# jrl-umi3218/jrl-walkgen

Hardware: AMD Instinct MI355X
Metric: QP-MPC ticks/sec (batch=4096, N=16) (higher is better)
Workload: dtype f64

## Files before the change

### include/wg_mpc.h

```cpp
#ifndef WG_MPC_H
#define WG_MPC_H

#include <stddef.h>

#ifdef __cplusplus
extern "C" {
#endif

#define WG_OK 0
#define WG_ERR_NO_DEVICE (-1)
#define WG_ERR_BAD_ARG (-2)
#define WG_ERR_HIP (-3)
#define WG_ERR_TOO_LARGE (-4)
#define WG_ERR_BUSY (-5)


int wg_init(int device_ordinal);
void wg_shutdown(void);
const char *wg_last_error(void);
int wg_abi_version(void);
size_t wg_qp_lds_bytes(int n, int m);

int wg_shard_range(long long total, int rank, int world, long long *lo, long long *hi);

// ... 88 lines not shown
  wg_foot_sample_t lf[WG_SAMPLES_PER_TICK], rf[WG_SAMPLES_PER_TICK];
  wg_foot_sample_t lf_back, rf_back;
  double pad_[15];
} wg_tick_out_t;

void wg_model_defaults(wg_model_t *model);

void wg_gait_init(const wg_model_t *model, wg_gait_state_t *state,
                  const double com0[3] , const double left_xyt[3],
                  const double right_xyt[3] );


int wg_mpc_configure(const wg_model_t *model);
int wg_mpc_reserve(int max_gaits);

int wg_mpc_tick_batch(int B, wg_gait_state_t *states, wg_tick_out_t *outs, int *diag, int advance_calls,
                      int *hist, int hist_cap, int *hist_len);
int wg_mpc_tick_batch_dev(int B, wg_gait_state_t *states, wg_tick_out_t *outs, int *diag, int advance_calls,
                          int *hist, int hist_cap, int *hist_len, void *hip_stream);
int wg_mpc_run_batch_dev(int B, wg_gait_state_t *states, int n_ticks, int advance_calls, wg_tick_out_t *outs, int *diag,
                         void *hip_stream);
int wg_mpc_run_sched_dev(int B, wg_gait_state_t *states, int n_ticks, int advance_calls, const double *vref_sched,
                         int period, wg_tick_out_t *outs, int *diag, void *hip_stream);
int wg_mpc_set_velref_dev(int B, wg_gait_state_t *states, const double *vref, void *hip_stream);
int wg_host_alloc(void **out, size_t bytes);
void wg_host_free(void *p);
int wg_mpc_tick_pinned(wg_gait_state_t *state, wg_tick_out_t *out, int *diag, int advance_calls);
int wg_mpc_assemble_batch(int B, const wg_gait_state_t *states, int advance_calls, int nmax, int mmax, double *C, double *d,
                          double *A, double *b, double *xl, double *xu, int *n, int *m);
int wg_mpc_assemble_batch_dev(int B, const wg_gait_state_t *states, int advance_calls, int nmax, int mmax, double *C, double *d,
                              double *A, double *b, double *xl, double *xu, int *n, int *m, void *hip_stream);
size_t wg_mpc_tick_lds_bytes(void);
size_t wg_mpc_tick_lds_bytes_for(const wg_model_t *model);

#define WG_RICCATI_WITH_INITIALPOS 0
#define WG_RICCATI_WITHOUT_INITIALPOS 1
int wg_riccati_solve(int n, const double *A, const double *b, const double *c, double Q, double R, int Nl, int mode,
                     double *K, double *F);
int wg_riccati_gains(double T, double zc, double Q, double R, int Nl, int mode, double *K, double *F);

#define WG_PLDP_N 16
#define WG_PLDP_MMAX (8 * WG_PLDP_N)
#define WG_PLDP_ACTIVE_CAP 40
#define WG_PLDP_NAN (-1)
#define WG_PLDP_NEG_ALPHA (-2)
#define WG_PLDP_CAPACITY (-3)
#define WG_PLDP_BAD_INPUT (-4)
typedef struct wg_pldp_state {
  int n_prev;
  int prev_active[WG_PLDP_MMAX];
  int pad_;
  double prev_zmp[2 * WG_PLDP_N];
  double internal_time;
} wg_pldp_state_t;
int wg_pldp_configure(int N, const double *iPu, const double *Px, const double *Pu);
int wg_pldp_solve_batch(int B, int mcap, const int *m, const double *D, const double *A, const double *b,
                        const double *zmpref, const double *xkyk, const int *similar, const int *n_removed,
                        const int *starting, int max_iter, wg_pldp_state_t *states, double *X, int *ret, int *n_iter,
                        int *active, int *n_active);
int wg_pldp_solve_batch_dev(int B, int mcap, const int *m, const double *D, const double *A, const double *b,
                            const double *zmpref, const double *xkyk, const int *similar, const int *n_removed,
                            const int *starting, int max_iter, wg_pldp_state_t *states, double *X, int *ret,
                            int *n_iter, int *active, int *n_active, void *hip_stream);
size_t wg_pldp_lds_bytes(void);

#define WG_POLY_MAX_ROWS 8
// ... 250 lines not shown
```

### jrl-walkgen_amd/csrc/wg_capi.hip

```cpp
#include <hip/hip_runtime.h>

#include <climits>
#include <cmath>
#include <cstdarg>
#include <cstdio>
#include <cstdlib>
#include <cstring>
#include <limits>
#include <memory>
#include <mutex>
#include <string>
#include <type_traits>
#include <vector>

#include "../../include/wg_mpc.h"
#include "wg_ql_device.hpp"
#include "wg_tick_device.hpp"
#include "wg_tick_kernels.hpp"
#include "wg_pldp_device.hpp"
#include "wg_dimitrov_device.hpp"
#include "wg_preview_device.hpp"
#include "wg_gramian_device.hpp"
#include "wg_zmpdisc_device.hpp"
#include "wg_footcons_device.hpp"
// ... 591 lines not shown
  const size_t lds = TickPlan(*model).lds;
  if (lds > 160 * 1024) return fail(WG_ERR_TOO_LARGE, "tick needs %zu B of LDS > 160 KiB", lds);
  std::vector<double> qb;
  if (model->flags & (WG_FLAG_GRAMIAN_MFMA_F64 | WG_FLAG_GRAMIAN_MFMA_F32)) {
    qb.resize((size_t)model->N * model->N);
    const int prec = (model->flags & WG_FLAG_GRAMIAN_MFMA_F32) ? WG_GRAMIAN_F32 : WG_GRAMIAN_F64;
    if (int rc = wg_gramian_batch_ctx(ctx, 1, model->N, &model->T, &model->com_height_qp, model->alpha, model->beta, model->gamma,
                                  prec, qb.data()))
      return rc;
  }
  std::lock_guard<std::mutex> lk(ctx->mu);
  std::unique_ptr<wg::TickTables> host_tables_p(new wg::TickTables);
  wg::TickTables &host_tables = *host_tables_p;
  wg::build_tables(*model, host_tables, qb.empty() ? nullptr : qb.data());
  if (!host_tables.blocks_ok && !qb.empty())
    return fail(WG_ERR_BAD_ARG, "the matrix-core Gramian is not positive definite enough for ql0002's factorisation");
  if (!ctx->tables_dev) HIP_TRY(hipMalloc(reinterpret_cast<void **>(&ctx->tables_dev), sizeof(wg::TickTables)));
  if (!ctx->model_dev) HIP_TRY(hipMalloc(reinterpret_cast<void **>(&ctx->model_dev), sizeof(wg_model_t)));
  if (int rc = ctx_wait_own(ctx)) return rc;
  HostScope hs(ctx);
  WG_H2D(ctx->tables_dev, &host_tables, sizeof host_tables);
  WG_H2D(ctx->model_dev, model, sizeof(wg_model_t));
  WG_HOST_WAIT();
  ctx->model = *model;
  ctx->model_set = true;
  return WG_OK;
}

size_t wg_mpc_tick_lds_bytes_for(const wg_model_t *model) {
  if (!model || model->N < 2 || model->N > wg::kNMaxH || tick_max_prw_steps(*model) > wg::kSMax) return 0;
  return TickPlan(*model).lds;
}

size_t wg_mpc_tick_lds_bytes_ctx(wg_ctx_t *ctx) {
  if (!ctx || !ctx->model_set) return 0;
  return TickPlan(ctx->model).lds;
}

int wg_mpc_reserve_ctx(wg_ctx_t *ctx, int max_gaits) {
  if (int rc = use_ctx(ctx)) return rc;
  if (!ctx->model_set) return fail(WG_ERR_BAD_ARG, "wg_mpc_configure() has not been called on this context");
  if (max_gaits < 1) return fail(WG_ERR_BAD_ARG, "max_gaits = %d", max_gaits);
  const TickPlan plan(ctx->model);
  std::lock_guard<std::mutex> launch_lk(ctx->launch_mu);
  double *zs = nullptr;
  if (int rc = plan.reserve_slots(ctx, max_gaits, &zs)) return rc;
  return ctx->run_buf.reserve(run_buf_bytes(max_gaits));
}

}
namespace {
int tick_launch(wg_ctx_t *ctx, int B, wg_gait_state_t *states, wg_tick_out_t *outs, int *diag, int advance_calls, int *hist, int hist_cap, int *hist_len, void *hip_stream, wg_gait_state_t *host_states, int *host_done) {
  if (int rc = tick_check(ctx, B, states)) return rc;
  if (hist && (!hist_len || hist_cap <= 0)) return fail(WG_ERR_BAD_ARG, "hist needs hist_len and hist_cap > 0");
  if (B == 0) return WG_OK;
  const TickPlan plan(ctx->model);
  if (int rc = plan.raise_lds(WG_KERNEL_BY_VIEW(wg_mpc_tick_kernel, plan.view))) return rc;
  const int grid = B;
  hipStream_t st = reinterpret_cast<hipStream_t>(hip_stream);
  std::lock_guard<std::mutex> launch_lk(ctx->launch_mu);
  if (int rc = slot_claim(ctx, ctx->guard_order, st, "tick / run")) return rc;
  double *zs = nullptr;
  if (int rc = plan.reserve_slots(ctx, grid, &zs)) return rc;
  int *order = nullptr, *iters_out = nullptr;
  if (B > ctx->num_cu * plan.per_cu() && !host_states && env_flag("WG_TICK_LPT", true))
    if (int rc = lpt_prepare(ctx->tick_lpt, states, B, st, &order, &iters_out)) return rc;
// ... 961 lines not shown
```

### jrl-walkgen_amd/csrc/wg_dimitrov_device.hpp

```cpp
#pragma once
#include "wg_pldp_device.hpp"

namespace wg {

struct DimitrovConst {
  int N, solver;
  double T, Tctrl, h;
  double OptB[2 * WG_PLDP_N * 6], OptC[2 * WG_PLDP_N * 2 * WG_PLDP_N], iLQ[2 * WG_PLDP_N * 2 * WG_PLDP_N];
  PldpModel pldp;
  double Qq[2 * WG_PLDP_N * 2 * WG_PLDP_N], OptBq[2 * WG_PLDP_N * 6], OptCq[2 * WG_PLDP_N * 2 * WG_PLDP_N], PuTq[WG_PLDP_N * WG_PLDP_N];
};

struct DimitrovHost {
  static void matmul(const double *A, const double *B, double *C, int r, int inner, int c) {
    for (int i = 0; i < r; i++)
      for (int j = 0; j < c; j++) {
        double s = 0.0;
        for (int k = 0; k < inner; k++) s += A[i * inner + k] * B[k * c + j];
        C[i * c + j] = s;
      }
  }
  static bool build(const wg_dimitrov_model_t &m, DimitrovConst &K) {
    const unsigned N = (unsigned)m.N, n = 2 * N;
    const double T = m.T;
// ... 179 lines not shown
      const double cy0 = xk[3] + t * xk[4] + 0.5 * t * t * xk[5] + t * t * t * jy / 6.0;
      const double cy1 = xk[4] + t * xk[5] + 0.5 * t * t * jy;
      const double cy2 = xk[5] + t * jy;
      out->com_x[lane][0] = cx0; out->com_x[lane][1] = cx1; out->com_x[lane][2] = cx2;
      out->com_y[lane][0] = cy0; out->com_y[lane][1] = cy1; out->com_y[lane][2] = cy2;
      out->zmp_x[lane] = 1.0 * cx0 + 0.0 * cx1 + c02 * cx2;
      out->zmp_y[lane] = 1.0 * cy0 + 0.0 * cy1 + c02 * cy2;
    }
    if (lane < 2) {
      const double T = K.T;
      const double A01 = T, A02 = T * T / 2.0, A12 = T, B0 = T * T * T / 6.0, B1 = T * T / 2.0, B2 = T;
      const double u = lane == 0 ? jx : jy;
      const double *c = xk + 3 * lane;
      const double n0 = 0.0 + 1.0 * c[0] + A01 * c[1] + A02 * c[2];
      const double n1 = 0.0 + 0.0 * c[0] + 1.0 * c[1] + A12 * c[2];
      const double n2 = 0.0 + 0.0 * c[0] + 0.0 * c[1] + 1.0 * c[2];
      st->xk[3 * lane + 0] = n0 + u * B0; st->xk[3 * lane + 1] = n1 + u * B1; st->xk[3 * lane + 2] = n2 + u * B2;
    }
  }
  if (lane == 0) {
    st->starting = 0;
    st->n_removed = first_rows;
    if (out) { out->jerk_x = jx; out->jerk_y = jy; out->ret = rc; out->n_iter = it; out->n_active = S; out->m = m; }
  }
  WG_WSYNC();
  return it;
}

template <bool kLQ>
struct DimitrovQldProb {
  static constexpr bool kCompact = false;
  static constexpr bool kNanExact = WG_TICK_NAN_EXACT != 0;
  static constexpr bool kHasFactor = false;
  static constexpr bool kRowOps = false;
  static constexpr bool kWideN = false;
  static constexpr int kFixedLdz = 0;
  static constexpr int kNM = 2 * WG_PLDP_N;
  const wg_zmp_polytope_t *polys;
  const int *slot;
  const int *rowbase;
  const double *PuT;
  int N;
  __device__ __forceinline__ double coef(int k, int inst, int axis) const { return polys[inst].A[k - rowbase[inst]][axis]; }
  __device__ __forceinline__ double G(const QlView &q, int i, int j) const {
    if constexpr (kLQ) return i == j ? q.Gdiag[i] : 0.0;
    else {
      const double g = q.G[i + j * q.ldg], dg = q.Gdiag[i];
      return i == j ? dg : g;
    }
  }
  __device__ __forceinline__ double Gd(const QlView &q, int i) const { return q.Gdiag[i]; }
  __device__ __forceinline__ void setGd(const QlView &q, int i, double v) const { q.Gdiag[i] = v; }
  __device__ __forceinline__ double xl(const QlView &, int) const { return -1e8; }
  __device__ __forceinline__ double xu(const QlView &, int) const { return 1e8; }
  __device__ __forceinline__ double A(const QlView &, int k, int i) const {
    const bool second = i >= N;
    const int kk = second ? i - N : i;
    const int inst = slot[k];
    const double a = coef(k, inst, second ? 1 : 0);
    if constexpr (kLQ) return a * PuT[kk * N + inst];
    else {
      const double pu = PuT[kk * N + (kk <= inst ? inst : kk)];
      return kk <= inst ? a * pu : 0.0;
    }
  }
  static constexpr bool kRegRows = true;
// ... 147 lines not shown
```

### jrl-walkgen_amd/csrc/wg_ql_device.hpp

```cpp
#pragma once
#include <hip/hip_runtime.h>

#include <type_traits>

#include "wg_wave.hpp"
#include "wg_ql_view.hpp"
#include "wg_ql_phases.hpp"

namespace wg {

#define WG_BACKSUB(q, s, nact, lane)                                                                   \
  do {                                                                                                 \
    if constexpr (P::kNM > 0 && P::kNM + 12 <= 48) backsub_lds<48>(q, s, nact, lane, q.sc0);          \
    else if (P::kNM == 0 && (P::kWideN || q.n >= 48) && (nact) <= 60) backsub_lds<96>(q, s, nact, lane, q.sc0);     \
    else if (P::kNM == 0 && !P::kRowOps && q.n >= 24 && (nact) <= 36) backsub_lds<48>(q, s, nact, lane, q.sc0); \
    else backsub(q, s, nact, lane);                                                                    \
  } while (0)
#define WG_SWEEP(q, s, nu, nact, lane) \
  do { if (P::kNM > 0 || (!P::kRowOps && q.n <= 64)) sweep_flat<P::kFixedLdz>(q, s, nu, nact, lane PT_SW_ARG); else sweep<(P::kRowOps ? WG_ELEM_GRP : 8), P::kWideN>(q, s, nu, nact, lane); } while (0)

#define QL_SCAN_ACCEPT                                                                        \
  if (wak <= 0.0) continue;                                                                   \
  double sumx = -sum * wak;                                                                   \
  if (k + 1 <= me) sumx = fabs(sumx);                                                         \
// ... 16 lines not shown
  const int maxit = (m + n) * 40;
  const double onha = 1.5, xmagr = .01, diagr = 2.0;
  const int ifinc = 3, kfinc = n > 10 ? n : 10;
  int jfinc = -kfinc;
  double xmag = 0.0, vfact = 1.0, res = 0.0, ratio = 0.0, diag = 0.0;
  double wsel = 1.0;
  int knext = 0;
  const int s_tail = q.r_tail;
  double *s = q.R + s_tail;
  bool early_exit = false;
  bool cap_hit = false;
  bool x_suspect = false;
  auto x_has_non_numbers = [&]() {
    bool b = false;
    for (int i = lane; i < n; i += 64) { const bool bi = !wg_sane(q.x[i]); b = b || bi; }
    return __ballot(b) != 0ull;
  };
  PT_DECL
  if (resuming) {
    nact = rs->nact; info = rs->info; iterc = rs->iterc; itref = rs->itref; iflag = rs->iflag; jfinc = rs->jfinc; knext = rs->knext;
    out.hist_len = rs->hist_len;
    xmag = rs->xmag; vfact = rs->vfact; res = rs->res; ratio = rs->ratio; diag = rs->diag;
    if constexpr (kNan) x_suspect = x_has_non_numbers();
  }

#define LOG_EVENT(code)                                                   \
  do {                                                                    \
    if (lane == 0 && hist && out.hist_len < hist_cap) hist[out.hist_len] = (code); \
    out.hist_len++;                                                       \
  } while (0)

  if (!resuming) {
    int fatal = 0x7fffffff;
    if constexpr (P::kCompact) {
      fatal = prob.norms(q, lane);
    } else {
      for (int k = lane; k < m; k += 64) {
        double sum = 0.0;
        if constexpr (P::kRowOps) sum = prob.row_sqnorm(q, k);
        else {
          WG_UNROLL
          for (int i = 0; i < n; ++i) { double a = Am(k, i); sum += a * a; }
        }
        if (sum > 0.0) sum = 1.0 / sqrt(sum);
        else if (q.b[k] == 0.0) {}
        else if (k + 1 <= me || !(q.b[k] <= 0.0)) fatal = k + 1 < fatal ? k + 1 : fatal;
        q.wa[k] = sum;
      }
    }
    for (int k = lane; k < n; k += 64) q.wa[m + k] = 1.0;
    fatal = uni(wave_min_int(fatal));
    if (fatal != 0x7fffffff) { info = -fatal; early_exit = true; }
  }
  PT(PS_NORMS);

  if (!early_exit && !resuming) {
    for (int i = lane; i < n; i += 64) q.wd[i] = prob.Gd(q, i);
    WG_WSYNC();
    if constexpr (P::kCompact) {
      diag = prob.diag_check(q, vsmall, lane);
    } else {
      double dl = 0.0;
      for (int i = lane; i < n; i += 64) {
        double wdi = q.wd[i];
        dl = maxd(dl, vsmall - wdi);
        WG_UNROLL
        for (int j = i + 1; j < n; ++j) {
          double gjj = q.wd[j], gij = Gm(i, j);
          double ga = -mind(wdi, gjj);
          double gb = fabs(wdi - gjj) + fabs(gij);
          if (gb > 0.0) ga += gij * gij / gb;
          dl = maxd(dl, ga);
        }
      }
      diag = wave_max(dl);
    }
    diag = uni(diag);
    bool need_shift = !(diag <= 0.0);
    PT(PS_DIAGCHK);
    bool factored = false;
    if constexpr (P::kHasFactor) {
      WG_REP(8)
      if (!need_shift && prob.blocks_ok) factored = WG_UBOOL(prob.factor(q, vsmall, lane));
    }
    if constexpr (P::kNM > 0 && P::kNM <= 64 && !P::kHasFactor) {
      if (!factored && !need_shift) factored = chol_inverse_regs<P::kNM>(q, prob, vsmall, lane);
    }
    if (!factored) {
    for (;;) {
      if (need_shift) {
        diag = diagr * diag;
        for (int i = lane; i < n; i += 64) prob.setGd(q, i, diag + q.wd[i]);
        WG_WSYNC();
      }
      int jfail = -1;
      double tfail = 0.0;
      for (int i = 0; i < n; ++i) {
        for (int j = i + lane; j < n; j += 64) {
          double temp = Gm(i, j);
          WG_UNROLL
          for (int k = 0; k < i; ++k) temp -= Rf(k, j) * Rf(k, i);
          if (j == i) {
            if (temp < vsmall) { q.slot[0] = 1.0; q.slot[1] = temp; }
            else { q.slot[0] = 0.0; Rf(i, i) = sqrt(temp); }
          } else q.sc0[j] = temp;
        }
        WG_WSYNC();
        if (WG_UBOOL(q.slot[0] != 0.0)) { jfail = i; tfail = q.slot[1]; break; }
// ... 653 lines not shown
```

### jrl-walkgen_amd/csrc/wg_ql_herdt.hpp

```cpp
#pragma once
#include "wg_ql_device.hpp"

namespace wg {

constexpr int kSMaxQ = 4;
constexpr int kGvLd = 4;
constexpr int kQbLd = 32;

template <int NH, int NS>
__device__ __forceinline__ bool herdt_border_rows(const QlView &q, const double *gd, const double *Gv, double vsmall, int lane) {
  constexpr int M2 = 2 * NH;
  const int i = lane;
  const bool jerk = i < NH, foot = i >= NH && i < NH + NS, row = jerk || foot;
  const int fi = i - NH;
  const int gi = jerk ? i : M2 + (foot ? fi : 0);
  double acc[NS];
#pragma unroll
  for (int f = 0; f < NS; ++f)
    acc[f] = (jerk || (foot && f >= fi)) ? ((foot && f == fi) ? gd[gi] : Gv[gi * kGvLd + f]) : 0.0;
  const double dreg = jerk ? Rf(i, i) : 1.0;
  const int colbase = jerk ? i * (i + 1) / 2 : 0;
  const int khi = jerk ? i : 0;
  double rnext = (0 < khi) ? q.Rf[colbase] : 0.0;
  for (int k = 0; k < NH; ++k) {
// ... 138 lines not shown
#pragma unroll
  for (int t = 0; t < TZ; ++t) { const int e = lane + 64 * t; zv[t] = e < NH * NH ? Z2[(e % NH) + (e / NH) * M2] : 0.0; }
#pragma unroll
  for (int t = 0; t < TR; ++t) {
    const int e = lane + 64 * t;
    if (e < NR) {
      int j = 0;
      while ((j + 1) * (j + 2) / 2 <= e) ++j;
      const int i = e - j * (j + 1) / 2;
      q.Rf[e] = rv[t];
      Rf(NH + i, NH + j) = rv[t];
    }
  }
  for (int e = lane; e < NH * NH; e += 64) { const int i = e % NH, j = NH + e / NH; Rf(i, j) = 0.0; }
#pragma unroll
  for (int t = 0; t < TZ; ++t) {
    const int e = lane + 64 * t;
    if (e < NH * NH) {
      const int i = e % NH, j = e / NH;
      Zm(i, j) = zv[t]; Zm(NH + i, NH + j) = zv[t];
      Zm(NH + i, j) = 0.0;
      Zm(i, NH + j) = ((z2sign[e >> 6] >> (e & 63)) & 1ull) ? wg_kconst(-0.0) : 0.0;
    }
  }
  for (int e = lane; e < (n - M2) * M2; e += 64) { const int i = M2 + e % (n - M2), j = e / (n - M2); Zm(i, j) = 0.0; }
}

template <int NH>
struct HerdtProb {
  static constexpr bool kCompact = true;
  static constexpr bool kNanExact = WG_TICK_NAN_EXACT != 0;
  static constexpr bool kHasFactor = true;
  static constexpr bool kRowOps = false;
  static constexpr int kNM = 2 * NH + 2 * 2;
  static constexpr int kCopRows = 4 * NH;
  static constexpr bool kWideN = false;
  static constexpr int kFixedLdz = kNM | 1;
  static_assert(4 * NH == 64, "one CoP row per lane needs 4N == 64");
  const double *Qb;
  const double *u;
  double *Gv;
  double *gd;
  const double *rowA, *rowB;
  const int *rowK, *stepidx;
  const double *V_f;
  const double *R2, *Z2;
  const unsigned long long *z2sign;
  double diag_b;
  int blocks_ok;
  int ns;
  double ax[NH], ay[NH];
  int fj;
  double ra, rb;
  double bcop;
  double ga, gb; int gk;
  __device__ __forceinline__ double fa() const { return ra + 0.0; }
  __device__ __forceinline__ double fb() const { return rb + 0.0; }
  struct FootRow { double v[4]; int c[4]; };
  __device__ __forceinline__ FootRow foot_row() const {
    const bool used = gk >= 0, pred = gk > 0;
    const int kk = used ? gk : 0;
    FootRow r;
    const int c1 = 2 * NH + kk, c3 = 2 * NH + ns + kk;
    r.c[0] = used ? (pred ? c1 - 1 : c1) : 2 * NH; r.c[1] = used ? c1 : 2 * NH;
    r.c[2] = used ? (pred ? c3 - 1 : c3) : 2 * NH; r.c[3] = used ? c3 : 2 * NH;
    r.v[0] = pred ? ga + 0.0 : 0.0; r.v[1] = used ? 0.0 - ga : 0.0;
// ... 310 lines not shown
  __device__ __forceinline__ void zt_row(const QlView &q, double *s, int rk, int lane) const {
    const int n = q.n;
    if (lane < n) {
      const int i = lane;
      const double *zc = q.Z + i * q.ldz;
      double acc = 0.0;
      if (rk >= 1 && rk <= 4 * NH) {
        constexpr int kZtChunk = 8;
        const int r = (rk - 1) >> 2;
#pragma unroll
        for (int j0 = 0; j0 < 2 * NH; j0 += kZtChunk) {
          if ((j0 < NH ? j0 : j0 - NH) > r) continue;
          double zz[kZtChunk], wv[kZtChunk];
#pragma unroll
          for (int c = 0; c < kZtChunk; ++c) { zz[c] = zc[j0 + c]; wv[c] = q.ww[j0 + c]; }
#pragma unroll
          for (int c = 0; c < kZtChunk; ++c) acc += zz[c] * wv[c];
        }
      }
      for (int j = 2 * NH; j < n; ++j) acc += zc[j] * q.ww[j];
      s[i] = acc;
    }
    WG_WSYNC();
  }
};

constexpr int kGvLdElem = kSMaxQ;
template <int NHC>
struct HerdtElemProbT {
  static constexpr bool kCompact = false;
  static constexpr bool kNanExact = WG_TICK_NAN_EXACT != 0;
  static constexpr bool kHasFactor = true;
  static constexpr bool kRowOps = true;
  static constexpr int kNM = 0;
  static constexpr bool kWideN = NHC >= 32;
  static constexpr int kFixedLdz = 0;
  static constexpr int kHorizon = NHC;
  struct NConst { static constexpr int v = NHC; __device__ __forceinline__ NConst &operator=(int) { return *this; } __device__ __forceinline__ operator int() const { return v; } };
  typename std::conditional<(NHC > 0), NConst, int>::type N;
  int ns;
  const double *Qb;
  const double *u;
  double *Gv;
  double *gd;
  const double *rowA, *rowB;
  const int *rowK, *stepidx;
  const double *V_f;
  const double *R2, *Z2;
  const unsigned long long *z2sign;
  int blocks_ok;
  __device__ __forceinline__ bool factor(const QlView &q, double vsmall, int lane) const {
    if ((int)N != 32 || ns < 1 || ns > 4) return false;
    constexpr int NHc = 32;
    herdt_constant_blocks<NHc>(q, R2, Z2, z2sign, lane);
    WG_WSYNC();
    bool ok = true;
    switch (ns) {
      case 1: ok = herdt_border_rows<NHc, 1>(q, gd, Gv, vsmall, lane); break;
      case 2: ok = herdt_border_rows<NHc, 2>(q, gd, Gv, vsmall, lane); break;
      case 3: ok = herdt_border_rows<NHc, 3>(q, gd, Gv, vsmall, lane); break;
      default: ok = herdt_border_rows<NHc, 4>(q, gd, Gv, vsmall, lane); break;
    }
    if (!WG_UBOOL(ok)) return false;
    WG_WSYNC();
    switch (ns) {
      case 1: herdt_border_z<NHc, 1>(q, lane); break;
      case 2: herdt_border_z<NHc, 2>(q, lane); break;
      case 3: herdt_border_z<NHc, 3>(q, lane); break;
      default: herdt_border_z<NHc, 4>(q, lane); break;
    }
    WG_WSYNC();
    return true;
  }
  __device__ __forceinline__ double G(const QlView &q, int i, int j) const {
    if (i == j) return gd[i];
    if (j < i) { const int t = i; i = j; j = t; }
    if (j < 2 * N) {
      if (i < N && j < N) return Qb[i * kQbLd + j];
      if (i >= N && j >= N) return Qb[(i - N) * kQbLd + (j - N)];
      return 0.0;
    }
    const int c = j - 2 * N;
    const bool xcol = c < ns, xrow = (i < N) || (i >= 2 * N && i < 2 * N + ns);
// ... 59 lines not shown
#define WG_SCAN_CH 4
#endif
      constexpr int CH = WG_SCAN_CH;
#pragma unroll 1
      for (int c0 = 0; c0 <= rmax; c0 += CH) {
        double vv[CH], uu[CH];
#pragma unroll
        for (int e = 0; e < CH; ++e) { const int d = r - c0 - e, ci = c0 + e < N ? c0 + e : N - 1; vv[e] = v[ci]; uu[e] = u[d > -1 ? d : -1]; }
#pragma unroll
        for (int e = 0; e < CH; ++e) { const double t = vv[e] * (0.0 - ac * uu[e]); sum += t; asum += fabs(t); }
      }
#pragma unroll 1
      for (int c0 = 0; c0 <= rmax; c0 += CH) {
        double vv[CH], uu[CH];
#pragma unroll
        for (int e = 0; e < CH; ++e) { const int d = r - c0 - e, ci = c0 + e < N ? c0 + e : N - 1; vv[e] = v[N + ci]; uu[e] = u[d > -1 ? d : -1]; }
#pragma unroll
        for (int e = 0; e < CH; ++e) { const double t = vv[e] * (0.0 - bc * uu[e]); sum += t; asum += fabs(t); }
      }
      const int j = (r >= 0) ? stepidx[r] - 1 : -1;
      const bool st = j >= 0 && j < ns;
      const int jc = st ? j : 0;
      { const double t = v[2 * N + jc] * ((st ? a : 0.0) * 1.0 + 0.0); sum += t; asum += fabs(t); }
      { const double t = v[2 * N + ns + jc] * ((st ? b : 0.0) * 1.0 + 0.0); sum += t; asum += fabs(t); }
    }
    if (k0 + 63 > 4 * N) {
      const bool ft = k > 4 * N && kk >= 0;
      const int kf = ft ? kk : 0;
      const double af = ft ? a : 0.0, bf = ft ? b : 0.0;
      for (int j = 0; j < ns; ++j) { const double t = v[2 * N + j] * (0.0 - af * V_f[kf * kSMaxQ + j]); sum += t; asum += fabs(t); }
      for (int j = 0; j < ns; ++j) { const double t = v[2 * N + ns + j] * (0.0 - bf * V_f[kf * kSMaxQ + j]); sum += t; asum += fabs(t); }
    }
  }
  __device__ __forceinline__ double row_sqnorm(const QlView &, int k) const {
    double sum = 0.0;
    if (k == 0) return sum;
    const double a = rowA[k], b = rowB[k];
    const int kk = rowK[k];
    if (k <= 4 * N) {
      const int r = kk;
      for (int c = 0; c <= r; ++c) { const double e = 0.0 + (0.0 + a * u[r - c]) * -1.0; sum += e * e; }
      for (int c = 0; c <= r; ++c) { const double e = 0.0 + (0.0 + b * u[r - c]) * -1.0; sum += e * e; }
      const int j = stepidx[r] - 1;
      if (j >= 0 && j < ns) {
        { const double e = 0.0 + (0.0 + a * 1.0) * 1.0; sum += e * e; }
        { const double e = 0.0 + (0.0 + b * 1.0) * 1.0; sum += e * e; }
      }
      return sum;
    }
    if (kk < 0) return sum;
    for (int j = 0; j < ns; ++j) { const double e = 0.0 + (0.0 + a * V_f[kk * kSMaxQ + j]) * -1.0; sum += e * e; }
    for (int j = 0; j < ns; ++j) { const double e = 0.0 + (0.0 + b * V_f[kk * kSMaxQ + j]) * -1.0; sum += e * e; }
    return sum;
  }
};
typedef HerdtElemProbT<-1> HerdtElemProb;

}
```

### jrl-walkgen_amd/csrc/wg_ql_view.hpp

```cpp
#pragma once
#include <hip/hip_runtime.h>

#include <type_traits>

#include "wg_wave.hpp"
#include "wg_prof.hpp"

namespace wg {

struct QlDims {
  int n, m, mmax;
  int ldg, ldz, lda;
  bool dense;
  bool a_lds;
  int nsc;
  bool bounds;
  bool z_lds;
  bool wab_lds;
  bool cold_lds;
  int r_cols;
  bool g_lds;
  __host__ __device__ QlDims(int n_, int m_, int mmax_, bool dense_ = true, bool a_lds_ = true, int nsc_ = 0,
                             bool bounds_ = true, bool z_lds_ = true, bool wab_lds_ = true, bool cold_lds_ = true, int r_cols_ = 0,
                             bool g_lds_ = true)
// ... 84 lines not shown
  }
  template <int NMAX, int MMAX>
  __device__ __forceinline__ void carve_fixed_dense(double *base, int n_, int m_, int me_, double *ext_wab) {
    n = n_; m = m_; me = me_; mn = m_ + n_; ldg = NMAX; ldz = NMAX | 1; lda = MMAX;
    r_tail = n_ * (n_ + 1) / 2; nact_cap = 0;
    double *p = base;
    Z = p; p += NMAX * (NMAX | 1);
    R = p; p += NMAX * (NMAX + 1) / 2 + NMAX; Rf = R;
    x = p; p += NMAX; d = p; p += NMAX; ww = p; p += NMAX; wd = p; p += NMAX; wx = p; p += NMAX; lam = p; p += NMAX;
    xl = p; p += NMAX; xu = p; p += NMAX;
    Gdiag = p; p += NMAX;
    wa = ext_wab; b = ext_wab + (MMAX + NMAX);
    sc0 = p; p += NMAX; sc1 = p; p += NMAX; sc2 = p; p += NMAX; sc3 = p; p += NMAX;
    slot = p; p += 8;
    iact = reinterpret_cast<int *>(p);
    G = nullptr; A = nullptr;
  }
  template <int NMAX> static constexpr size_t fixed_dense_bytes() {
    return 8 * (size_t)(NMAX * (NMAX | 1) + NMAX * (NMAX + 1) / 2 + NMAX + 9 * NMAX + 4 * NMAX + 8) + 4 * (size_t)((NMAX + 1) & ~1);
  }
  template <int NMAX> static constexpr int fixed_elem_head() { return 3 * NMAX + 8 + ((NMAX + 1) & ~1) / 2; }
};

#define Zm(i, j) q.Z[(i) + (j) * q.ldz]
#define Gm(i, j) prob.G(q, (i), (j))
#define Am(k, i) prob.A(q, (k), (i))

struct QlView;
template <bool kGLds, int kNMc = 0>
struct DenseProbT {
  static constexpr bool kCompact = false;
  static constexpr bool kNanExact = true;
  static constexpr bool kHasFactor = false;
  static constexpr bool kRowOps = false;
  static constexpr int kNM = kNMc;
  static constexpr bool kWideN = false;
  static constexpr int kFixedLdz = kNMc > 0 ? (kNMc | 1) : 0;
  __device__ __forceinline__ double G(const QlView &q, int i, int j) const;
  __device__ __forceinline__ double A(const QlView &q, int k, int i) const;
  __device__ __forceinline__ double Gd(const QlView &q, int i) const;
  __device__ __forceinline__ void setGd(const QlView &q, int i, double v) const;
  __device__ __forceinline__ double xl(const QlView &q, int i) const;
  __device__ __forceinline__ double xu(const QlView &q, int i) const;
};
typedef DenseProbT<true> DenseProb;
template <int NM, int MM>
struct DenseRegProb : DenseProbT<false, NM> {
  static constexpr bool kRegRows = true;
  double ar0[NM], ar1[NM];
  __device__ __forceinline__ void load_rows(const QlView &q, int lane) {
    const int m = q.m;
    const int mc = m > 0 ? m - 1 : 0;
    const int k0 = lane < m ? lane : mc, k1 = lane + 64 < m ? lane + 64 : mc;
#pragma unroll
    for (int i = 0; i < NM; ++i) { ar0[i] = q.A[k0 + i * q.lda]; ar1[i] = q.A[k1 + i * q.lda]; }
  }
  __device__ __forceinline__ void row_to(const QlView &q, int k, double *dst, int lane) const {
    const int n = q.n;
    if (lane == (k & 63)) {
#pragma unroll
      for (int i = 0; i < NM; ++i)
        if (i < n) dst[i] = k < 64 ? ar0[i] : ar1[i];
    }
  }
};
template <class P, class = void> struct HasRegRows { static constexpr bool value = false; };
// ... 44 lines not shown
```

### jrl-walkgen_amd/csrc/wg_tick_device.hpp

```cpp
#pragma once
#include <hip/hip_runtime.h>

#include <cmath>

#include "../../include/wg_mpc.h"
#define WG_TRIG_FN __host__ __device__ static inline
#include "../../include/wg_trig.h"
#include "wg_ql_device.hpp"
#include "wg_ql_herdt.hpp"

namespace wg {

#define GmL(i, j) q.G[(i) + (j) * q.ldg]
#define AmL(k, i) q.A[(k) + (i) * q.lda]
#define WG_STATE_COPY(to, from)                                                                                       \
  { double *dst = reinterpret_cast<double *>(to); const double *src = reinterpret_cast<const double *>(from);          \
    for (int i = lane; i < (int)(sizeof(wg_gait_state_t) / 8); i += 64) dst[i] = src[i]; }
#define WG_STATE_COPY_LD(to, from, scope)                                                                              \
  { const double *src = reinterpret_cast<const double *>(from); double *dst = reinterpret_cast<double *>(to);           \
    for (int i = lane; i < (int)(sizeof(wg_gait_state_t) / 8); i += 64) dst[i] = __hip_atomic_load(src + i, __ATOMIC_RELAXED, scope); }

constexpr int kNMaxH = 32;
constexpr int kSMax = 4;
constexpr double kPi = 3.14159265358979323846;
// ... 749 lines not shown
    q.b[r] = -bacc;
  }
  WG_WSYNC();
  }

  TK(PS_TICK_ASSEMBLY);
  QlResult qr;
  if constexpr (kCompactView) {
    if (lane == 0 && fabs(L.gd[n - 1]) == 0.0) L.gd[n - 1] = wg_kconst(1e-8);
    WG_WSYNC();
    WG_STATE_COPY(gstate, s);
    HerdtProb<16> prob;
    prob.Qb = &tb->Qb[0][0]; prob.u = L.uvec; prob.Gv = L.Gv; prob.gd = L.gd;
    prob.rowA = L.rowA; prob.rowB = L.rowB; prob.rowK = L.rowK; prob.stepidx = L.stepidx; prob.V_f = L.V_f;
    prob.R2 = tb->R2; prob.Z2 = tb->Z2; prob.z2sign = tb->z2_cross_sign; prob.diag_b = tb->diag_b; prob.blocks_ok = tb->blocks_ok; prob.ns = ns;
    prob.load_rows(lane, q.b);
    qr = ql_solve(q, prob, 1e-8, hist, hist_cap);
    {
      WG_WSYNC();
      __builtin_amdgcn_fence(__ATOMIC_RELEASE, "workgroup");
      WG_STATE_COPY_LD(s, gstate, __HIP_MEMORY_SCOPE_AGENT);
      WG_WSYNC();
    }
  } else if constexpr (kElem) {
    if (lane == 0 && fabs(L.gd[n - 1]) == 0.0) L.gd[n - 1] = 1e-8;
    WG_WSYNC();
    {
      WG_STATE_COPY(gstate, s);
      __builtin_amdgcn_fence(__ATOMIC_RELEASE, "workgroup");
    }
    HerdtElemProbT<(NH == 32) ? 32 : -1> prob;
    prob.N = N; prob.ns = ns; prob.Qb = &tb->Qb[0][0]; prob.u = L.uvec; prob.Gv = L.Gv; prob.gd = L.gd;
    prob.rowA = L.rowA; prob.rowB = L.rowB; prob.rowK = L.rowK; prob.stepidx = L.stepidx; prob.V_f = L.V_f;
    prob.R2 = tb->R2; prob.Z2 = tb->Z2; prob.z2sign = tb->z2_cross_sign; prob.blocks_ok = tb->blocks_ok;
    QlResume rs;
    qr = ql_solve(q, prob, 1e-8, hist, hist_cap, &rs);
    if (WG_UBOOL(qr.ifail == kQlCapHit)) {
      WG_WSYNC();
      double *Rg = extE + eRfull;
      const int cnt = qr.nact * (qr.nact + 1) / 2;
      for (int i = lane; i < cnt; i += 64) Rg[i] = q.R[i];
      __builtin_amdgcn_fence(__ATOMIC_RELEASE, "workgroup");
      WG_WSYNC();
      q.R = Rg; q.Rf = q.R;
      q.r_tail = n * (n + 1) / 2;
      q.nact_cap = 0;
      rs.valid = 1;
      qr = ql_solve(q, prob, 1e-8, hist, hist_cap, &rs);
    }
    {
      WG_WSYNC();
      __builtin_amdgcn_fence(__ATOMIC_RELEASE, "workgroup");
      WG_STATE_COPY_LD(s, gstate, __HIP_MEMORY_SCOPE_AGENT);
      WG_WSYNC();
    }
  } else {
    if (dump) {
      const QpDumpOut &o = *dump;
      for (int e = lane; e < o.nmax * o.nmax; e += 64) { const int i = e % o.nmax, j = e / o.nmax; o.C[e] = (i < n && j < n) ? GmL(i, j) : 0.0; }
      for (int e = lane; e < o.mmax * o.nmax; e += 64) { const int k = e % o.mmax, i = e / o.mmax; o.A[e] = (k < mq && i < n) ? AmL(k, i) : 0.0; }
      for (int i = lane; i < o.nmax; i += 64) { o.d[i] = i < n ? q.d[i] : 0.0; o.xl[i] = i < n ? q.xl[i] : 0.0; o.xu[i] = i < n ? q.xu[i] : 0.0; }
      for (int k = lane; k < o.mmax; k += 64) o.b[k] = k < mq ? -q.b[k] : 0.0;
      if (lane == 0) { *o.n = n; *o.m = mq; }
      TickDiag dg0;
      dg0.ifail = 0; dg0.n_iter = 0; dg0.nact = 0; dg0.n = n; dg0.m = mq; dg0.ns = ns;
      return dg0;
    }
// ... 221 lines not shown
```

### jrl-walkgen_amd/wgmpc.py

```python
import ctypes as C
import os

import numpy as np

_HERE = os.path.dirname(os.path.abspath(__file__))
LIB_PATH = os.environ.get("WG_LIB_PATH", os.path.join(_HERE, "lib", "libwg_mpc.so"))

SAMPLES = 20


class FootSample(C.Structure):
    _fields_ = [(k, C.c_double) for k in
                ("x", "y", "z", "theta", "omega", "omega2", "dx", "dy", "dz", "dtheta", "domega", "domega2",
                 "ddx", "ddy", "ddz", "ddtheta", "ddomega", "ddomega2")]


class Model(C.Structure):
    _fields_ = [("N", C.c_int), ("flags", C.c_int)] + [(k, C.c_double) for k in
                ("T", "Tctrl", "com_height_qp", "alpha", "beta", "gamma", "sole_w", "sole_h", "margin_x", "margin_y",
                 "ds_feet_distance", "hip_l_lo", "hip_l_hi", "hip_r_lo", "hip_r_hi", "hip_vmax", "hip_amax",
                 "feet_cross_max", "step_period", "ds_period", "dsss_period", "t_single", "t_double", "step_height",
                 "feet_distance")]


# ... 260 lines not shown
    return dict(x=x, u=u, ifail=ifail, n_iter=n_iter, iact=iact, nact=nact, hist=hist, hist_len=hist_len)


def qp_solve_batch_dev(B, nmax, mmax, n, m, me, Cd, d, A, b, xl, xu, eps, x, u, ifail, n_iter=None, iact=None,
                       nact=None, hist=None, hist_cap=0, hist_len=None, stream=None):
    p = lambda t: None if t is None else C.c_void_p(t.data_ptr())
    rc = lib().wg_qp_solve_batch_dev(B, nmax, mmax, p(n), p(m), p(me), p(Cd), p(d), p(A), p(b), p(xl), p(xu), eps,
                                     p(x), p(u), p(ifail), p(n_iter), p(iact), p(nact), p(hist), hist_cap,
                                     p(hist_len), C.c_void_p(stream) if stream else None)
    _check(rc)


def model_defaults():
    m = Model()
    lib().wg_model_defaults(C.byref(m))
    return m


def gait_init(model, com0, left_xyt, right_xyt):
    s = GaitState()
    a3 = lambda v: (C.c_double * 3)(*v)
    lib().wg_gait_init(C.byref(model), C.byref(s), a3(com0), a3(left_xyt), a3(right_xyt))
    return s


def mpc_configure(model):
    _check(lib().wg_mpc_configure(C.byref(model)))


def mpc_tick_lds_bytes_for(model):
    return int(lib().wg_mpc_tick_lds_bytes_for(C.byref(model)))


def mpc_tick_lds_bytes():
    return int(lib().wg_mpc_tick_lds_bytes())


def mpc_tick_batch(states, want_out=True, advance_calls=0, hist_cap=0):
    B = len(states)
    outs = (TickOut * B)() if want_out else None
    diag = np.zeros((B, 6), dtype=np.int32)
    hist = np.zeros((B, hist_cap), dtype=np.int32) if hist_cap else None
    hlen = np.zeros(B, dtype=np.int32) if hist_cap else None
    rc = lib().wg_mpc_tick_batch(B, C.addressof(states), C.addressof(outs) if outs is not None else None, _hp(diag),
                                 advance_calls, _hp(hist), hist_cap, _hp(hlen))
    _check(rc)
    return outs, diag, hist, hlen


def mpc_assemble_batch(states, advance_calls=0, nmax=None, mmax=None, model=None):
    B = len(states)
    N = model.N if model is not None else 16
    nmax = nmax or 2 * N + 8
    mmax = mmax or 1 + 4 * N + 20 + 1
    Cb = np.zeros((B, nmax * nmax)); Ab = np.zeros((B, mmax * nmax)); d = np.zeros((B, nmax)); b = np.zeros((B, mmax))
    xl = np.zeros((B, nmax)); xu = np.zeros((B, nmax)); n = np.zeros(B, dtype=np.int32); m = np.zeros(B, dtype=np.int32)
    _check(lib().wg_mpc_assemble_batch(B, C.addressof(states), int(advance_calls), nmax, mmax, _hp(Cb), _hp(d), _hp(Ab), _hp(b),
                                       _hp(xl), _hp(xu), _hp(n), _hp(m)))
    return dict(B=B, nmax=nmax, mmax=mmax, n=n, m=m, me=np.zeros(B, dtype=np.int32), C=Cb, d=d, A=Ab, b=b, xl=xl, xu=xu)


class HostMapped:

    def __init__(self):
        p = C.c_void_p()
        size = C.sizeof(GaitState) + C.sizeof(TickOut) + 64
# ... 367 lines not shown
```

Measured before the change: 6.586 million.

## Precompute Gramian diagonal-dominance bound and vectorise row-norm pass for Herdt elem QP

Adds a host-precomputed diagonal bound (diag_b) so the QL diagonal shift check only scans the step-variable tail of the Hessian instead of all pairs, when the table bound applies. Replaces the per-row scalar row_sqnorm with a wave-wide norms routine that prefetches row coefficients for three 64-row passes and branchlessly accumulates CoP and foot-constraint row norms. A test entry point exposes the table bound. The skipped pairwise scan relies on the precomputed bound being valid, and the new norm code adds more registers.

```diff
diff --git a/include/wg_mpc.h b/include/wg_mpc.h
--- a/include/wg_mpc.h
+++ b/include/wg_mpc.h
@@ -144,6 +144,7 @@
                               double *A, double *b, double *xl, double *xu, int *n, int *m, void *hip_stream);
 size_t wg_mpc_tick_lds_bytes(void);
 size_t wg_mpc_tick_lds_bytes_for(const wg_model_t *model);
+int wg_mpc_diag_test_for(const wg_model_t *model, double *diag_b, int *blocks_ok);
 
 #define WG_RICCATI_WITH_INITIALPOS 0
 #define WG_RICCATI_WITHOUT_INITIALPOS 1
diff --git a/jrl-walkgen_amd/csrc/wg_capi.hip b/jrl-walkgen_amd/csrc/wg_capi.hip
--- a/jrl-walkgen_amd/csrc/wg_capi.hip
+++ b/jrl-walkgen_amd/csrc/wg_capi.hip
@@ -647,6 +647,15 @@
   return TickPlan(*model).lds;
 }
 
+int wg_mpc_diag_test_for(const wg_model_t *model, double *diag_b, int *blocks_ok) {
+  if (!model || model->N < 2 || model->N > wg::kNMaxH) return fail(WG_ERR_BAD_ARG, "null model or N outside [2,%d]", wg::kNMaxH);
+  std::unique_ptr<wg::TickTables> t(new wg::TickTables);
+  wg::build_tables(*model, *t);
+  if (diag_b) *diag_b = t->diag_b;
+  if (blocks_ok) *blocks_ok = t->blocks_ok;
+  return WG_OK;
+}
+
 size_t wg_mpc_tick_lds_bytes_ctx(wg_ctx_t *ctx) {
   if (!ctx || !ctx->model_set) return 0;
   return TickPlan(ctx->model).lds;
diff --git a/jrl-walkgen_amd/csrc/wg_dimitrov_device.hpp b/jrl-walkgen_amd/csrc/wg_dimitrov_device.hpp
--- a/jrl-walkgen_amd/csrc/wg_dimitrov_device.hpp
+++ b/jrl-walkgen_amd/csrc/wg_dimitrov_device.hpp
@@ -235,6 +235,8 @@
   static constexpr bool kCompact = false;
   static constexpr bool kNanExact = WG_TICK_NAN_EXACT != 0;
   static constexpr bool kHasFactor = false;
+  static constexpr bool kHasDiagCheck = false;
+  static constexpr bool kDiagCheckAlways = false;
   static constexpr bool kRowOps = false;
   static constexpr bool kWideN = false;
   static constexpr int kFixedLdz = 0;
diff --git a/jrl-walkgen_amd/csrc/wg_ql_device.hpp b/jrl-walkgen_amd/csrc/wg_ql_device.hpp
--- a/jrl-walkgen_amd/csrc/wg_ql_device.hpp
+++ b/jrl-walkgen_amd/csrc/wg_ql_device.hpp
@@ -72,16 +72,13 @@
 
   if (!resuming) {
     int fatal = 0x7fffffff;
-    if constexpr (P::kCompact) {
+    if constexpr (P::kCompact || P::kRowOps) {
       fatal = prob.norms(q, lane);
     } else {
       for (int k = lane; k < m; k += 64) {
         double sum = 0.0;
-        if constexpr (P::kRowOps) sum = prob.row_sqnorm(q, k);
-        else {
-          WG_UNROLL
-          for (int i = 0; i < n; ++i) { double a = Am(k, i); sum += a * a; }
-        }
+        WG_UNROLL
+        for (int i = 0; i < n; ++i) { double a = Am(k, i); sum += a * a; }
         if (sum > 0.0) sum = 1.0 / sqrt(sum);
         else if (q.b[k] == 0.0) {}
         else if (k + 1 <= me || !(q.b[k] <= 0.0)) fatal = k + 1 < fatal ? k + 1 : fatal;
@@ -97,9 +94,14 @@
   if (!early_exit && !resuming) {
     for (int i = lane; i < n; i += 64) q.wd[i] = prob.Gd(q, i);
     WG_WSYNC();
-    if constexpr (P::kCompact) {
+    if constexpr (P::kHasDiagCheck && P::kDiagCheckAlways) {
       diag = prob.diag_check(q, vsmall, lane);
     } else {
+      bool tabled = false;
+      if constexpr (P::kHasDiagCheck) {
+        if (WG_UBOOL(prob.diag_applies())) { diag = prob.diag_check(q, vsmall, lane); tabled = true; }
+      }
+      if (!tabled) {
       double dl = 0.0;
       for (int i = lane; i < n; i += 64) {
         double wdi = q.wd[i];
@@ -114,6 +116,7 @@
         }
       }
       diag = wave_max(dl);
+      }
     }
     diag = uni(diag);
     bool need_shift = !(diag <= 0.0);
diff --git a/jrl-walkgen_amd/csrc/wg_ql_herdt.hpp b/jrl-walkgen_amd/csrc/wg_ql_herdt.hpp
--- a/jrl-walkgen_amd/csrc/wg_ql_herdt.hpp
+++ b/jrl-walkgen_amd/csrc/wg_ql_herdt.hpp
@@ -194,6 +194,8 @@
   static constexpr bool kNanExact = WG_TICK_NAN_EXACT != 0;
   static constexpr bool kHasFactor = true;
   static constexpr bool kRowOps = false;
+  static constexpr bool kHasDiagCheck = true;
+  static constexpr bool kDiagCheckAlways = true;
   static constexpr int kNM = 2 * NH + 2 * 2;
   static constexpr int kCopRows = 4 * NH;
   static constexpr bool kWideN = false;
@@ -570,6 +572,8 @@
   static constexpr bool kNanExact = WG_TICK_NAN_EXACT != 0;
   static constexpr bool kHasFactor = true;
   static constexpr bool kRowOps = true;
+  static constexpr bool kHasDiagCheck = true;
+  static constexpr bool kDiagCheckAlways = false;
   static constexpr int kNM = 0;
   static constexpr bool kWideN = NHC >= 32;
   static constexpr int kFixedLdz = 0;
@@ -586,7 +590,9 @@
   const double *V_f;
   const double *R2, *Z2;
   const unsigned long long *z2sign;
+  double diag_b;
   int blocks_ok;
+  int diag_ok;
   __device__ __forceinline__ bool factor(const QlView &q, double vsmall, int lane) const {
     if ((int)N != 32 || ns < 1 || ns > 4) return false;
     constexpr int NHc = 32;
@@ -712,26 +718,91 @@
       for (int j = 0; j < ns; ++j) { const double t = v[2 * N + ns + j] * (0.0 - bf * V_f[kf * kSMaxQ + j]); sum += t; asum += fabs(t); }
     }
   }
-  __device__ __forceinline__ double row_sqnorm(const QlView &, int k) const {
-    double sum = 0.0;
-    if (k == 0) return sum;
-    const double a = rowA[k], b = rowB[k];
-    const int kk = rowK[k];
-    if (k <= 4 * N) {
-      const int r = kk;
-      for (int c = 0; c <= r; ++c) { const double e = 0.0 + (0.0 + a * u[r - c]) * -1.0; sum += e * e; }
-      for (int c = 0; c <= r; ++c) { const double e = 0.0 + (0.0 + b * u[r - c]) * -1.0; sum += e * e; }
-      const int j = stepidx[r] - 1;
-      if (j >= 0 && j < ns) {
-        { const double e = 0.0 + (0.0 + a * 1.0) * 1.0; sum += e * e; }
-        { const double e = 0.0 + (0.0 + b * 1.0) * 1.0; sum += e * e; }
-      }
-      return sum;
-    }
-    if (kk < 0) return sum;
-    for (int j = 0; j < ns; ++j) { const double e = 0.0 + (0.0 + a * V_f[kk * kSMaxQ + j]) * -1.0; sum += e * e; }
-    for (int j = 0; j < ns; ++j) { const double e = 0.0 + (0.0 + b * V_f[kk * kSMaxQ + j]) * -1.0; sum += e * e; }
-    return sum;
+  __device__ __forceinline__ int norms(const QlView &q, int lane) const {
+    const int m = q.m, me = q.me;
+    int fatal = 0x7fffffff;
+    constexpr int kNormPasses = 3;
+    double ra_p[kNormPasses], rb_p[kNormPasses], bk_p[kNormPasses];
+    int rk_p[kNormPasses];
+#pragma unroll
+    for (int pp = 0; pp < kNormPasses; ++pp) {
+      const int k = 1 + 64 * pp + lane;
+      const int kc = k < m ? k : 0;
+      ra_p[pp] = rowA[kc]; rb_p[pp] = rowB[kc]; rk_p[pp] = rowK[kc]; bk_p[pp] = q.b[kc];
+    }
+#pragma unroll
+    for (int pp = 0; pp < kNormPasses; ++pp) {
+      const int k0 = 1 + 64 * pp;
+      if (k0 >= m) break;
+      const int k = k0 + lane;
+      const bool in = k < m;
+      const int kc = in ? k : 0;
+      const double a = ra_p[pp], b = rb_p[pp];
+      const int kk = rk_p[pp];
+      double sum = 0.0;
+      if (k0 <= 4 * N) {
+        const bool cop = kc >= 1 && kc <= 4 * N;
+        const int r = cop ? kk : -1;
+        const int klast = (k0 + 63 < 4 * N) ? k0 + 63 : 4 * N;
+        const int rmax = (klast - 1) >> 2;
+        constexpr int CH = 4;
+#pragma unroll 1
+        for (int c0 = 0; c0 <= rmax; c0 += CH) {
+          double uu[CH];
+#pragma unroll
+          for (int e = 0; e < CH; ++e) { const int d = r - c0 - e; uu[e] = u[d > -1 ? d : -1]; }
+#pragma unroll
+          for (int e = 0; e < CH; ++e) { const double t = 0.0 - a * uu[e]; const double el = (r - c0 - e >= 0) ? t : 0.0; sum += el * el; }
+        }
+#pragma unroll 1
+        for (int c0 = 0; c0 <= rmax; c0 += CH) {
+          double uu[CH];
+#pragma unroll
+          for (int e = 0; e < CH; ++e) { const int d = r - c0 - e; uu[e] = u[d > -1 ? d : -1]; }
+#pragma unroll
+          for (int e = 0; e < CH; ++e) { const double t = 0.0 - b * uu[e]; const double el = (r - c0 - e >= 0) ? t : 0.0; sum += el * el; }
+        }
+        const int j = (r >= 0) ? stepidx[r] - 1 : -1;
+        const bool st = j >= 0 && j < ns;
+        { const double el = st ? a : 0.0; sum += el * el; }
+        { const double el = st ? b : 0.0; sum += el * el; }
+      }
+      if (k0 + 63 > 4 * N) {
+        const bool ft = kc > 4 * N && kk >= 0;
+        const int kf = ft ? kk : 0;
+        for (int j = 0; j < ns; ++j) { const double t = 0.0 - a * V_f[kf * kSMaxQ + j]; const double el = ft ? t : 0.0; sum += el * el; }
+        for (int j = 0; j < ns; ++j) { const double t = 0.0 - b * V_f[kf * kSMaxQ + j]; const double el = ft ? t : 0.0; sum += el * el; }
+      }
+      if (in) {
+        const double bk = bk_p[pp];
+        if (sum > 0.0) sum = 1.0 / sqrt(sum);
+        else if (bk == 0.0) {}
+        else if (k + 1 <= me || !(bk <= 0.0)) fatal = k + 1 < fatal ? k + 1 : fatal;
+        q.wa[k] = sum;
+      }
+    }
+    if (lane == 0) q.wa[0] = 0.0;
+    return fatal;
+  }
+
+  __device__ __forceinline__ bool diag_applies() const { return diag_ok != 0; }
+  __device__ __forceinline__ double diag_check(const QlView &q, double vsmall, int lane) const {
+    const int n = q.n;
+    const int M2 = 2 * N;
+    double dl = diag_b;
+    for (int i = lane; i < n; i += 64) {
+      const double wdi = q.wd[i];
+      if (i >= M2) dl = maxd(dl, vsmall - wdi);
+      const int j0 = (i + 1 > M2) ? i + 1 : M2;
+      for (int j = j0; j < n; ++j) {
+        const double gjj = q.wd[j], gij = G(q, i, j);
+        double ga = -mind(wdi, gjj);
+        const double gb = fabs(wdi - gjj) + fabs(gij);
+        if (gb > 0.0) ga += gij * gij / gb;
+        dl = maxd(dl, ga);
+      }
+    }
+    return wave_max(dl);
   }
 };
 typedef HerdtElemProbT<-1> HerdtElemProb;
diff --git a/jrl-walkgen_amd/csrc/wg_ql_view.hpp b/jrl-walkgen_amd/csrc/wg_ql_view.hpp
--- a/jrl-walkgen_amd/csrc/wg_ql_view.hpp
+++ b/jrl-walkgen_amd/csrc/wg_ql_view.hpp
@@ -140,6 +140,8 @@
   static constexpr bool kCompact = false;
   static constexpr bool kNanExact = true;
   static constexpr bool kHasFactor = false;
+  static constexpr bool kHasDiagCheck = false;
+  static constexpr bool kDiagCheckAlways = false;
   static constexpr bool kRowOps = false;
   static constexpr int kNM = kNMc;
   static constexpr bool kWideN = false;
diff --git a/jrl-walkgen_amd/csrc/wg_tick_device.hpp b/jrl-walkgen_amd/csrc/wg_tick_device.hpp
--- a/jrl-walkgen_amd/csrc/wg_tick_device.hpp
+++ b/jrl-walkgen_amd/csrc/wg_tick_device.hpp
@@ -805,7 +805,8 @@
     HerdtElemProbT<(NH == 32) ? 32 : -1> prob;
     prob.N = N; prob.ns = ns; prob.Qb = &tb->Qb[0][0]; prob.u = L.uvec; prob.Gv = L.Gv; prob.gd = L.gd;
     prob.rowA = L.rowA; prob.rowB = L.rowB; prob.rowK = L.rowK; prob.stepidx = L.stepidx; prob.V_f = L.V_f;
-    prob.R2 = tb->R2; prob.Z2 = tb->Z2; prob.z2sign = tb->z2_cross_sign; prob.blocks_ok = tb->blocks_ok;
+    prob.R2 = tb->R2; prob.Z2 = tb->Z2; prob.z2sign = tb->z2_cross_sign; prob.diag_b = tb->diag_b; prob.blocks_ok = tb->blocks_ok;
+    prob.diag_ok = ((ns > 0 || !(fabs(tb->Qb[N - 1][N - 1]) == 0.0)) && tb->diag_b == tb->diag_b) ? 1 : 0;
     QlResume rs;
     qr = ql_solve(q, prob, 1e-8, hist, hist_cap, &rs);
     if (WG_UBOOL(qr.ifail == kQlCapHit)) {
diff --git a/jrl-walkgen_amd/wgmpc.py b/jrl-walkgen_amd/wgmpc.py
--- a/jrl-walkgen_amd/wgmpc.py
+++ b/jrl-walkgen_amd/wgmpc.py
@@ -316,6 +316,14 @@
     return int(lib().wg_mpc_tick_lds_bytes_for(C.byref(model)))
 
 
+def mpc_diag_test_for(model):
+    d, ok = C.c_double(0.0), C.c_int(0)
+    f = lib().wg_mpc_diag_test_for
+    f.restype, f.argtypes = C.c_int, [C.c_void_p, C.c_void_p, C.c_void_p]
+    _check(f(C.byref(model), C.byref(d), C.byref(ok)))
+    return d.value, ok.value
+
+
 def mpc_tick_lds_bytes():
     return int(lib().wg_mpc_tick_lds_bytes())
 
```

After: 6.585 million. No clear change (-0.0%).
